# tlk00/BitMagic

Measured on AMD Instinct MI355X. Metric: Gbits/s + % HBM roofline, 256-way fused AND+COUNT on 1B-bit vectors, higher is better.
Workload: dtype u64; 1 GPU; aggregator pipeline combine_and_sub counts-only: 256-way AND+COUNT, 256 x 1000000000-bit vectors in total, data set A (common 10% OR noise 10%: no early exit); vectors=256, bits_per_vector=1000000000, density_q16=6554, blocks_per_vector=15259, blocks_per_rank=15259, hbm_resident_bytes=32279432448

## Files before the change

bitmagic_amd/_ffi.py:

```python
from __future__ import annotations

import ctypes as C
import os

_HERE = os.path.dirname(os.path.abspath(__file__))
LIB_PATH = os.environ.get("BMX_LIB") or os.path.join(_HERE, "lib", "libbmx.so")

OK, ERR_BADALLOC, ERR_BADARG, ERR_RANGE, ERR_DEVICE = 0, 1, 2, 3, 4
RC_BATCH_MAX = 8


class BmxError(RuntimeError):
    def __init__(self, status: int, msg: str, detail: str):
        super().__init__(f"{msg}" + (f" [{detail}]" if detail else ""))
        self.status = status


_lib = None


def lib() -> C.CDLL:
    global _lib
    if _lib is not None:
        return _lib
# ... 146 lines not shown
        "bmx_timer_stop_ms": (i32, [vp, P(C.c_float)]),
    }
    missing = []
    for name, (res, args) in sig.items():
        try:
            fn = getattr(L, name)
        except AttributeError:
            missing.append(name)
            continue
        fn.restype, fn.argtypes = res, args
    if missing:
        raise ImportError(f"libbmx.so does not export: {', '.join(missing)}")
    if hasattr(L, "bmx_diag_stream_read"):
        L.bmx_diag_stream_read.restype = i32
        L.bmx_diag_stream_read.argtypes = [vp, u64, i32, u32, i32, i32, P(C.c_float)]
    _lib = L
    return L


def exported_symbols():
    import re
    hdr = os.path.join(os.path.dirname(_HERE), "include", "bmx.h")
    txt = open(hdr).read()
    return sorted(set(re.findall(r"\b(bmx_[a-z0-9_]+)\s*\(", txt)))


def check(status: int) -> None:
    if status != OK:
        L = lib()
        raise BmxError(status, L.bmx_error_msg(status).decode(), L.bmx_last_error().decode())
# ... 1 lines not shown
```

bitmagic_amd/csrc/bmx.hip:

```cpp
#include "bmx_internal.h"
#ifdef BMX_DIAG
#include "bmx_diag.h"
#endif
#include "bmx_kernels2.h"
#include "bmx_kernels3.h"
#include "bmx_kernels4.h"
#include "bmx_kernels5.h"
#include "bmx_kernels6.h"
#include "bmx_kernels7.h"
#include "bmx_kernels8.h"
#include "bmx_kernels9.h"
#include "bmx_kernels10.h"
#include "bmx_kernels11.h"
#include "bmx_kernels12.h"
#include "bmx_kernels13.h"
#include "bmx_kernels14.h"
#include "bmx_kernels15.h"
#include "bmx_kernels16.h"
#include "bmx_kernels17.h"
#include "bmx_kernels18.h"

#include <algorithm>
#include <atomic>
#include <chrono>
// ... 734 lines not shown
#endif
#undef B2
    return nullptr;
}
static pipe_bits_fn pipe_bits_kernel(u32 rows, u32 unroll, bool nt, u32 wg)
{
    switch (rows) {
    case 8: return pipe_bits_rows<8>(unroll, nt, wg);
    case 4: return pipe_bits_rows<4>(unroll, nt, wg);
    case 2: return pipe_bits_rows<2>(unroll, nt, wg);
    case 1: return pipe_bits_rows<1>(unroll, nt, wg);
    default: return nullptr;
    }
}

static int ctx_set_tuning(bmx_ctx* ctx, const char* key, int value)
{
    ARGCHK(ctx && key);
    std::string k(key);
    if (k == "pipe_unroll") { ARGCHK(value == 0 || value == 1 || value == 2 || value == 4 || value == 8 || value == 16); ctx->pipe_unroll = value; }
    else if (k == "pipe_rows") { ARGCHK(value == 0 || value == 8 || value == 4 || value == 2 || value == 1); ctx->pipe_rows = value; }
    else if (k == "pipe_nt") ctx->pipe_nt = value != 0;
    else if (k == "pipe_lds") { ARGCHK(value >= 0 && value <= 160 * 1024); ctx->pipe_lds = value; }
    else if (k == "pipe_slots") { ARGCHK(value == 8 || value == 16); ctx->pipe_slots = value; }
    else if (k == "pipe_staged") { ARGCHK(value >= -1 && value <= 1); ctx->pipe_staged = value; }
    else if (k == "pipe_split") { ARGCHK(value >= -1 && value <= 1); ctx->pipe_split = value; }
    else if (k == "pipe_window") { ARGCHK(value >= -1); ctx->pipe_window = value; }
    else if (k == "or_tile") { ARGCHK(value >= 0 && value <= 3); ctx->or_tile = value; }
    else if (k == "or_rows") { ARGCHK(value >= -1 && value <= 1); ctx->or_rows = value; }
    else if (k == "or_depth") { ARGCHK(value == 4 || value == 8); ctx->or_depth = value; }
    else if (k == "direct_cols") { ARGCHK(value >= 0); ctx->direct_cols = value; }
    else if (k == "pair_stream") { ARGCHK(value == -1 || value == 0 || value == 2 || value == 4 || value == 8); ctx->pair_stream = value; }
    else if (k == "pair_wgs") { ARGCHK(value >= 1 && value <= 8); ctx->pair_wgs = value; }
    else if (k == "range_halves") { ARGCHK(value == 0 || value == 1); ctx->range_halves = value; }
    else if (k == "gap_count") { ARGCHK(value >= -1 && value <= 1); ctx->gap_count = value; }
    else if (k == "agg_shape") { ARGCHK(value == 0 || value == 1); ctx->agg_shape = value; }
    else if (k == "and_rows") { ARGCHK(value >= -1 && value <= 1); ctx->and_rows = value; }
    else if (k == "and_rows_wg") { ARGCHK(value == 128 || value == 256 || value == 512); ctx->and_rows_wg = value; }
    else if (k == "and_rows_depth") { ARGCHK(value == 2 || value == 3 || value == 4 || value == 8); ctx->and_rows_depth = value; }
    else if (k == "and_rows_nt") ctx->and_rows_nt = value != 0;
    else if (k == "and_rows_ipw") { ARGCHK(value >= 0 && value <= 64); ctx->and_rows_ipw = value; }
    else if (k == "ff_window") { ARGCHK(value >= -1); ctx->ff_window = value; }
// ... 151 lines not shown
    HIPCHK(hipMemsetAsync(ctx->d_done, 0, FOLD_DONE_WORDS * 4, ctx->stream));
    HIPCHK(hipMalloc((void**)&ctx->d_slots2, COUNT_SLOTS * COUNT_SLOT_STRIDE * sizeof(u64)));
    HIPCHK(hipMemsetAsync(ctx->d_slots2, 0, COUNT_SLOTS * COUNT_SLOT_STRIDE * sizeof(u64), ctx->stream));
    HIPCHK(hipMalloc((void**)&ctx->d_done2, FOLD_DONE_WORDS * 4));
    HIPCHK(hipMemsetAsync(ctx->d_done2, 0, FOLD_DONE_WORDS * 4, ctx->stream));
    HIPCHK(hipHostMalloc((void**)&ctx->h_pend, PEND_SLOTS * 8 * sizeof(u64)));
    HIPCHK(hipMalloc((void**)&ctx->d_cursor, 64));
    HIPCHK(hipMemsetAsync(ctx->d_cursor, 0, 64, ctx->stream));
    { int v = 0; if (hipDeviceGetAttribute(&v, hipDeviceAttributeMaxSharedMemoryPerBlock, device) == hipSuccess && v > 0) ctx->max_lds_bytes = (uint32_t)v; else (void)hipGetLastError(); }
    { size_t fr = 0, tot = 0; if (hipMemGetInfo(&fr, &tot) == hipSuccess && fr) ctx->pack_cap = (uint64_t)fr / 4; else (void)hipGetLastError(); }
    if (const char* e = getenv("BMX_DEBUG_REDZONE")) ctx->redzone = atoi(e) != 0;
    if (const char* e = getenv("BMX_PACK_MAX_MB")) { long long mb = atoll(e); if (mb >= 0) ctx->pack_cap = (uint64_t)mb << 20; }
    if (const char* e = getenv("BMX_POOL_MAX_MB")) { long long mb = atoll(e); if (mb >= 0) ctx->pool_cap = (uint64_t)mb << 20; }
    static const char* const env_keys[][2] = {
        {"BMX_PIPE_UNROLL", "pipe_unroll"}, {"BMX_PIPE_ROWS", "pipe_rows"}, {"BMX_PIPE_NT", "pipe_nt"},
        {"BMX_PIPE_WG", "pipe_wg"}, {"BMX_PIPE_WINDOW", "pipe_window"}, {"BMX_PIPE_SPLIT", "pipe_split"}, {"BMX_OR_TILE", "or_tile"}, {"BMX_OR_ROWS", "or_rows"}, {"BMX_OR_DEPTH", "or_depth"}, {"BMX_OR_WINDOW", "or_window"}, {"BMX_DIRECT_COLS", "direct_cols"}, {"BMX_FF_WINDOW", "ff_window"}, {"BMX_RC_BATCH", "rc_batch"}, {"BMX_GAP_COUNT", "gap_count"}, {"BMX_AND_ROWS", "and_rows"}, {"BMX_AGG_SHAPE", "agg_shape"}, {"BMX_AND_ROWS_WG", "and_rows_wg"}, {"BMX_AND_ROWS_DEPTH", "and_rows_depth"}, {"BMX_AND_ROWS_NT", "and_rows_nt"}, {"BMX_AND_ROWS_IPW", "and_rows_ipw"}, {"BMX_RANGE_HALVES", "range_halves"}, {"BMX_PAIR_STREAM", "pair_stream"}, {"BMX_PAIR_WGS", "pair_wgs"}, {"BMX_RS_LANES", "rs_lanes"}, {"BMX_RS_SELECT_TOP", "rs_select_top"}, {"BMX_RS_SELECT_SEL", "rs_select_sel"}, {"BMX_RS_LINES", "rs_lines"}, {"BMX_RS_SELECT_LINES", "rs_select_lines"}, {"BMX_RS_SDIR_SHIFT", "rs_sdir_shift"}, {"BMX_COLL_SHAPE", "coll_shape"}, {"BMX_COLL_WINDOW", "coll_window"}, {"BMX_COLL_SPLIT", "coll_split"}, {"BMX_COLL_BUILD", "coll_build"}, {"BMX_EQ_BIG", "eq_big"}, {"BMX_PAIR_LOOP", "pair_loop"}, {"BMX_PAIR_NT", "pair_nt"}, {"BMX_EQ_BIG_SHAPE", "eq_big_shape"}, {"BMX_OP2_WGS", "op2_wgs"}, {"BMX_OP2_LOOP", "op2_loop"}, {"BMX_OP2_NT", "op2_nt"}, {"BMX_GAP_PACK", "gap_pack"}, {"BMX_COLL_MEMBERS", "coll_members"}, {"BMX_XCD_SWIZZLE", "xcd_swizzle"}, {"BMX_RANKC_PATH", "rankc_path"}, {"BMX_HITS_TABLE_KB", "hits_table_kb"}};
    for (auto& kv : env_keys)
        if (const char* e = getenv(kv[0])) (void)ctx_set_tuning(ctx.get(), kv[1], atoi(e));
    g_last_error.clear();
    *out = ctx.release();
    return BMX_OK;
ABI_END }

int bmx_ctx_destroy(bmx_ctx* ctx) { ABI_TRY if (ctx) ctx_release(ctx); return BMX_OK; ABI_END }

int bmx_ctx_set_tuning(bmx_ctx* ctx, const char* key, int value) { ABI_TRY return ctx_set_tuning(ctx, key, value); ABI_END }

int bmx_probe_stream_rw(bmx_ctx* ctx, uint64_t bytes, int sets, int wgs_per_cu, int iters, float* ms_per_pass)
{ ABI_TRY
    ARGCHK(ctx && ms_per_pass && bytes >= 8192 && sets >= 1 && sets <= 8 && wgs_per_cu >= 1 && wgs_per_cu <= 8 && iters >= 1);
    int rc = set_dev(ctx); if (rc) return rc;
// ... 1226 lines not shown
        }
        return BMX_OK;
    }
    case CK_AND_ROWS:
        hipLaunchKernelGGL(and_rows_kernel<AR_COUNT>(ctx), dim3((u32)((pl.nitems + pl.ar_ipw - 1u) / pl.ar_ipw)), dim3(pl.ar_wg), pl.lds, ctx->stream,
                           (const u64*)p->d_dmat, row_off, and_n, sub_n, p->col_stride, ngroups, nb_from, (u32)pl.nitems, ctx->xcd_swz, (u64*)d_counts,
                           (uint4*)nullptr, (u64*)nullptr, (BlockStat*)nullptr, 0u, 0xFFFFFFFFu, and_rows_diag_bits(), pl.ar_ipw);
        break;
    case CK_GAPCOUNT:
        HIPCHK(hipFuncSetAttribute(reinterpret_cast<const void*>(k_pipe_counts_gapcount<false>), hipFuncAttributeMaxDynamicSharedMemorySize, (int)pl.lds));
        hipLaunchKernelGGL(HIP_KERNEL_NAME(k_pipe_counts_gapcount<false>), dim3((u32)pl.nitems), dim3(1024), pl.lds, ctx->stream,
                           p->d_dmat, row_off, and_n, sub_n, p->col_stride, ngroups, nb_from, (u32)pl.nitems, (u64*)d_counts,
                           (uint4*)nullptr, (u64*)nullptr, (BlockStat*)nullptr, 0u, 0xFFFFFFFFu);
        break;
    case CK_GENERAL: {
        auto fn = k_pipe_counts<1>;
        if (pl.unroll != 1) fn = pl.unroll == 2 ? k_pipe_counts<2> : k_pipe_counts<4>;
        for (u32 c0 = 0; c0 < pl.ncols; c0 += pl.win.per) {
            u32 nitems = std::min(pl.win.per, pl.ncols - c0) * ngroups;
            hipLaunchKernelGGL(fn, dim3((nitems + 3) / 4), dim3(256), pl.lds, ctx->stream,
                               p->d_dmat, row_off, and_n, sub_n, p->col_stride, ngroups, nb_from + c0, nitems, ctx->xcd_swz, (u64*)d_counts);
            KCHK();
        }
        return BMX_OK;
    }
    }
    KCHK();
    return BMX_OK;
}

extern "C" {

int bmx_pipeline_describe(bmx_ctx* ctx, bmx_pipeline* p, uint32_t nb_from, uint32_t nb_to, char* buf, size_t buf_len, uint32_t* n_launches)
{ ABI_TRY
    ARGCHK(ctx && p && p->ctx == ctx && buf && buf_len > 0);
    if (n_launches) *n_launches = 1;
    int rc = pipe_range(p, nb_from, nb_to); if (rc) return rc;
    bmx_coll *ca = nullptr, *cs = nullptr;
    if (!p->h_uids.empty() && ctx->gap_pack != 0 && p->cm_gen == ctx->coll_gen) (void)pipe_colls_valid(ctx, p, &ca, &cs);
    const CountsPlan pl = counts_plan(ctx, p, nb_from, nb_to, p->ngroups, coll_serve(p, ca));
    switch (pl.kernel) {
    case CK_COLL_APPLY: snprintf(buf, buf_len, "k_coll_apply<AND_COUNT,512> x 1 launch, %llu workgroups (packed collection of the operand set)", pl.nitems); break;
    case CK_COLL_MEMBERS: snprintf(buf, buf_len, "k_coll_members<AND_COUNT> x 1 launch, a wave per (column, group): %u x %u items (members of a packed collection)", pl.ncols, pl.ngroups); break;
    case CK_STAGED: snprintf(buf, buf_len, "k_pipe_counts_staged<%u> x 1 launch, %u workgroups", pl.slots, pl.ncols); break;
    case CK_SPLIT: snprintf(buf, buf_len, "k_pipe_split<2,%d> x 1 launch, %llu workgroups", SPLIT_WAVES, pl.nitems); break;
    case CK_AND_ROWS: snprintf(buf, buf_len, "k_agg_and_rows<COUNT,%u,%u> x 1 launch, %llu workgroups", pl.ar_wg, pl.ar_depth, pl.nitems); break;
// ... 2431 lines not shown
```

bitmagic_amd/csrc/bmx_device.h:

```cpp
#pragma once
#include <hip/hip_runtime.h>
#include <stdint.h>

typedef uint8_t  u8;
typedef uint16_t u16;
typedef uint32_t u32;
typedef uint64_t u64;

#define GMETA(e) ((u32)((e) >> 48) & 0x1FFFu)
#define GMETA_NONE 0xFFFFFFFFu
#define BMX_DESC_KIND(d) ((u32)((d) & 3ull))
#define BMX_DESC_PTR(d)  ((d) & ~3ull)

typedef u32 u32x4 __attribute__((ext_vector_type(4)));
typedef const __attribute__((address_space(1))) u32x4* gcptr4;
typedef __attribute__((address_space(1))) u32x4* gptr4;
typedef const __attribute__((address_space(1))) u16* gcptr16;

template <int ROWS> struct Part { u32x4 r[ROWS]; };
typedef Part<8> Blk;

__device__ __forceinline__ gcptr4 as_gc4(u64 addr) { return (gcptr4)(uintptr_t)addr; }
__device__ __forceinline__ gcptr4 as_gc4(const void* p) { return (gcptr4)(uintptr_t)p; }
__device__ __forceinline__ gptr4 as_g4(void* p) { return (gptr4)(uintptr_t)p; }
// ... 435 lines not shown
    const u32x4* l4 = reinterpret_cast<const u32x4*>(lds);
    u32 c = 0;
#pragma unroll
    for (int i = 0; i < 8; ++i) {
        u32x4 t = l4[i * 64 + lane];
        c += (u32)__popc(t.x) + (u32)__popc(t.y) + (u32)__popc(t.z) + (u32)__popc(t.w);
    }
    return uniform32(wave_sum(c));
}

#define SPARSE_CAP 1024u
#define SPARSE_NONE 0xFFFFFFFFu

struct GapStage { u32x4 d[3]; };

__device__ __forceinline__ void gap_stage_load(GapStage& s, gcptr16 g, u32 hdr, u32 lane)
{
    gcptr4 g4 = (gcptr4)(uintptr_t)g;
    u32 nch = ((hdr >> 3) + 8u) >> 3;
    const u32x4 z = {0u, 0u, 0u, 0u};
#pragma unroll
    for (int j = 0; j < 3; ++j) { u32 c = lane + 64u * (u32)j; s.d[j] = c < nch ? g4[c] : z; }
}
__device__ __forceinline__ void gap_stage_store(const GapStage& s, u32* lds, u32 hdr, u32 lane)
{
    u32x4* l4 = reinterpret_cast<u32x4*>(lds);
    u32 nch = ((hdr >> 3) + 8u) >> 3;
#pragma unroll
    for (int j = 0; j < 3; ++j) { u32 c = lane + 64u * (u32)j; if (c < nch) l4[c] = s.d[j]; }
}

template <int MODE, int NJ>
__device__ __forceinline__ u32 sparse_test(u32 (&cand)[16], const u16* G, u32 hdr)
{
    u32 len = hdr >> 3, sbit = hdr & 1u;
    u32 k[NJ];
#pragma unroll
    for (int j = 0; j < NJ; ++j) k[j] = 0u;
    for (u32 step = 1u << (31 - __builtin_clz(len)); step; step >>= 1) {
#pragma unroll
        for (int j = 0; j < NJ; ++j) {
            u32 t = k[j] + step; t = t < len ? t : len;
            u32 v = G[t];
            k[j] = v < cand[j] ? t : k[j];
        }
    }
#pragma unroll
    for (int j = 0; j < NJ; ++j) {
        u32 bitv = (sbit ^ k[j]) & 1u;
        bool keep = (MODE == GAP_AND) ? (bitv != 0u) : (bitv == 0u);
        if (!keep) cand[j] = SPARSE_NONE;
    }
    u32 alive = 0;
#pragma unroll
    for (int j = 0; j < NJ; ++j) alive += (u32)__popcll(__ballot(cand[j] != SPARSE_NONE));
    return alive;
}

template <int MODE>
__device__ __forceinline__ bool gap_apply_sparse(const u64* __restrict__ plist_back, u32 i0, u32 n, u32* lds, u32 lane)
{
    u16* list = reinterpret_cast<u16*>(lds + 640);
    u32 cand[16];
    u32 total, nj;
    {
        Blk b; blk_from_lds(b, lds, lane);
        __builtin_amdgcn_fence(__ATOMIC_ACQ_REL, "wavefront");
        __builtin_amdgcn_wave_barrier();
        u32 cnt = blk_lane_popcount(b);
        u32 incl = wave_scan_incl(cnt, lane);
        total = uniform32(__shfl(incl, 63, 64));
        u32 off = incl - cnt;
#pragma unroll
        for (int i = 0; i < 8; ++i) {
            u32 ws[4] = {b.r[i].x, b.r[i].y, b.r[i].z, b.r[i].w};
#pragma unroll
            for (int c = 0; c < 4; ++c) {
                u32 w = ws[c];
                u32 base = ((u32)i * 256u + lane * 4u + (u32)c) << 5;
                while (w) { u32 bit = (u32)__builtin_ctz(w); w &= w - 1u; list[off++] = (u16)(base + bit); }
            }
        }
        __builtin_amdgcn_fence(__ATOMIC_ACQ_REL, "wavefront");
        __builtin_amdgcn_wave_barrier();
        nj = (total + 63u) >> 6;
#pragma unroll
        for (int j = 0; j < 16; ++j) {
            u32 idx = (u32)j * 64u + lane;
            cand[j] = idx < total ? (u32)list[idx] : SPARSE_NONE;
        }
    }
    const u16* G = reinterpret_cast<const u16*>(lds);
    u32 i = i0;
    gcptr16 g0 = as_gc16(uniform64(*(plist_back - i)));
    u32 h0 = uniform32((u32)g0[0]);
    GapStage cur; gap_stage_load(cur, g0, h0, lane);
    gcptr16 g1 = as_gc16(uniform64(*(plist_back - (i + 1u < n ? i + 1u : n - 1u))));
    u32 h1v = (u32)g1[0];
    for (; i < n; ++i) {
        u32 h1 = uniform32(h1v);
        GapStage nxt; gap_stage_load(nxt, g1, h1, lane);
        u32 i2 = i + 2u < n ? i + 2u : n - 1u;
        gcptr16 g2 = as_gc16(uniform64(*(plist_back - i2)));
        u32 h2v = (u32)g2[0];
        gap_stage_store(cur, lds, h0, lane);
        __builtin_amdgcn_fence(__ATOMIC_ACQ_REL, "wavefront");
        __builtin_amdgcn_wave_barrier();
        u32 alive;
        if (nj <= 1u) alive = sparse_test<MODE, 1>(cand, G, h0);
        else if (nj <= 2u) alive = sparse_test<MODE, 2>(cand, G, h0);
        else if (nj <= 3u) alive = sparse_test<MODE, 3>(cand, G, h0);
        else if (nj <= 4u) alive = sparse_test<MODE, 4>(cand, G, h0);
        else if (nj <= 6u) alive = sparse_test<MODE, 6>(cand, G, h0);
        else if (nj <= 8u) alive = sparse_test<MODE, 8>(cand, G, h0);
        else if (nj <= 12u) alive = sparse_test<MODE, 12>(cand, G, h0);
        else alive = sparse_test<MODE, 16>(cand, G, h0);
        if (alive == 0u) return true;
        if (((alive + 63u) >> 6) < nj) {
            u32 mine = 0;
#pragma unroll
            for (int j = 0; j < 16; ++j) mine += cand[j] != SPARSE_NONE ? 1u : 0u;
            u32 off = wave_scan_incl(mine, lane) - mine;
#pragma unroll
            for (int j = 0; j < 16; ++j) if (cand[j] != SPARSE_NONE) list[off++] = (u16)cand[j];
            __builtin_amdgcn_fence(__ATOMIC_ACQ_REL, "wavefront");
            __builtin_amdgcn_wave_barrier();
            nj = (alive + 63u) >> 6;
#pragma unroll
            for (int j = 0; j < 16; ++j) {
                u32 idx = (u32)j * 64u + lane;
                cand[j] = idx < alive ? (u32)list[idx] : SPARSE_NONE;
            }
        }
        __builtin_amdgcn_fence(__ATOMIC_ACQ_REL, "wavefront");
        __builtin_amdgcn_wave_barrier();
        cur = nxt; g0 = g1; h0 = h1; g1 = g2; h1v = h2v;
    }
    {
        u32x4* l4 = reinterpret_cast<u32x4*>(lds);
        const u32x4 z = {0u, 0u, 0u, 0u};
#pragma unroll
        for (int r = 0; r < 8; ++r) l4[r * 64 + lane] = z;
        __builtin_amdgcn_fence(__ATOMIC_ACQ_REL, "wavefront");
        __builtin_amdgcn_wave_barrier();
#pragma unroll
        for (int j = 0; j < 16; ++j)
            if (cand[j] != SPARSE_NONE) atomicOr(&lds[cand[j] >> 5], 1u << (cand[j] & 31u));
        __builtin_amdgcn_fence(__ATOMIC_ACQ_REL, "wavefront");
        __builtin_amdgcn_wave_barrier();
    }
    return false;
}

template <int MODE>
__device__ __forceinline__ bool gap_apply_list(const u64* __restrict__ plist_back, u32 n, u32* lds, u32 lane)
{
    const bool CHECK = MODE != GAP_OR;
    u32 head = n >= 32u ? 8u : n;
    u32 i = 0;
    if constexpr (CHECK) {
        if (n >= 2u) {
            u32 pop = lds_blk_popcount(lds, lane);
            if (pop == 0u) return true;
            if (pop <= SPARSE_CAP) return gap_apply_sparse<MODE>(plist_back, 0u, n, lds, lane);
        }
    }
    for (; i < head; ++i) {
        gap_apply_lds_wave<MODE>(as_gc16(uniform64(*(plist_back - i))), lds, lane);
        if constexpr (CHECK) {
            __builtin_amdgcn_fence(__ATOMIC_ACQ_REL, "wavefront");
            __builtin_amdgcn_wave_barrier();
            u32 pop = lds_blk_popcount(lds, lane);
            if (pop == 0u) return true;
            if (pop <= SPARSE_CAP && i + 2u < n) return gap_apply_sparse<MODE>(plist_back, i + 1u, n, lds, lane);
        }
    }
    if (i < n) {
        u64 p = i + lane < n ? *(plist_back - (i + lane)) : 0ull;
        for (; i < n; i += 64u) {
            u64 pn = i + 64u + lane < n ? *(plist_back - (i + 64u + lane)) : 0ull;
            if (i + lane < n) gap_apply_lds_lane<MODE>(as_gc16(p), lds);
            p = pn;
            if constexpr (CHECK) {
                __builtin_amdgcn_fence(__ATOMIC_ACQ_REL, "wavefront");
                __builtin_amdgcn_wave_barrier();
                u32 pop = lds_blk_popcount(lds, lane);
                if (pop == 0u) return true;
                if (pop <= SPARSE_CAP && i + 64u + 2u <= n)
                    return gap_apply_sparse<MODE>(plist_back, i + 64u, n, lds, lane);
            }
        }
    }
    __builtin_amdgcn_fence(__ATOMIC_ACQ_REL, "wavefront");
    __builtin_amdgcn_wave_barrier();
    return false;
}

__device__ __forceinline__ u32 gap_lane_popcount(gcptr16 g, u32 lane, u32 meta = GMETA_NONE)
{
    u32 len, s;
    if (meta != GMETA_NONE) { len = meta >> 1; s = meta & 1u; }
    else { u32 hdr = g[0]; len = hdr >> 3; s = hdr & 1u; }
    u32 c = 0;
    for (u32 k = 1 + lane; k <= len; k += 64) {
// ... 75 lines not shown
```

bitmagic_amd/csrc/bmx_diag.h:

```cpp
#pragma once
#include "../../include/bmx.h"
#ifdef __cplusplus
extern "C" {
#endif
int bmx_diag_stream_read(bmx_ctx* ctx, uint64_t bytes, int nontemporal, uint32_t blocks_per_wave,
                         int pattern ,
                         int iters, float* ms_per_pass);
#ifdef __cplusplus
}
#endif
```

bitmagic_amd/csrc/bmx_internal.h:

```cpp
#pragma once
#include "../../include/bmx.h"
#include <hip/hip_runtime.h>
#include <stdint.h>

#include <map>
#include <memory>
#include <string>
#include <unordered_map>
#include <vector>

typedef uint8_t  u8;
typedef uint16_t u16;
typedef uint32_t u32;
typedef uint64_t u64;

int bmx_fail_hip(hipError_t e, const char* what, const char* file, int line);
void bmx_set_last_error(const char* msg);
#define HIPCHK(call) do { hipError_t e_ = (call); if (e_ != hipSuccess) return bmx_fail_hip(e_, #call, __FILE__, __LINE__); } while (0)
#define ARGCHK(cond) do { if (!(cond)) { bmx_set_last_error("bad argument: " #cond); return BMX_ERR_BADARG; } } while (0)
#define KCHK() HIPCHK(hipGetLastError())
#define PEND_SLOTS 1024
#include <new>
#include <stdexcept>
int bmx_abi_caught(int kind, const char* what);
// ... 24 lines not shown
    hipEvent_t ev_stage = nullptr;
    std::multimap<size_t, void*> pool_free;
    std::unordered_map<void*, size_t> pool_live;
    uint64_t pool_cached = 0, pool_cap = 16ull << 30;
    struct RzInfo { void* raw; size_t block; size_t bytes; int line; };
    bool redzone = false;
    std::unordered_map<void*, RzInfo> rz_live;
    uint64_t rz_hits = 0; std::string rz_report;
    long long fail_dmalloc_after = -1;
    bool fail_dmalloc_throws = false;
    int pipe_unroll = 0;
    int pipe_rows = 0;
    int pipe_nt = 1;
    int pipe_wg = 0;
    int pipe_window = 0;
    int pipe_staged = -1;
    int pipe_lds = 0;
    int pipe_slots = 16;
    int pipe_split = -1;
    int or_tile = 0;
    int direct_cols = 384;
    int pair_stream = -1;
    int pair_wgs = 1;
    int range_halves = 1;
    int gap_count = -1;
    int agg_shape = 0;
    int and_rows = -1;
    int and_rows_wg = 256;
    int and_rows_ipw = 0;
    int and_rows_nt = 0;
// ... 140 lines not shown
```

bitmagic_amd/csrc/bmx_kernels.h:

```cpp
#pragma once
#include "bmx_device.h"

#define DESC_MAKE(ptr, kind) ((u64)(uintptr_t)(ptr) | ((u64)(kind) << 62))
#define DESC_K(d) ((u32)((d) >> 62))
#define DESC_P(d) ((d) & 0x0000FFFFFFFFFFFFull)
#define DESC_MAKE_GAP(ptr, len, sbit) (DESC_MAKE(ptr, K_GAP) | ((u64)((((u32)(len)) << 1) | ((u32)(sbit) & 1u)) << 48))
enum { K_NULL = 0, K_FULL = 1, K_BIT = 2, K_GAP = 3 };

#define ROW_EMPTY 1ull
#define ROW_FULL  2ull
#define ROW_ONES  4ull

struct BlockStat { u32 pop; u32 runs; u32 first; u32 kind; };

__global__ __launch_bounds__(256)
void k_generate(u64 seed, u32 vec_id, int with_common, u32 d, u64 nbits, u64* __restrict__ out, u64 nwords64, u64 word0)
{
    u64 i = (u64)blockIdx.x * blockDim.x + threadIdx.x;
    u64 stride = (u64)gridDim.x * blockDim.x;
    for (; i < nwords64; i += stride) {
        u64 w = word0 + i;
        u64 v = gen_word64(seed, vec_id, w, d);
        if (with_common) v |= gen_word64(seed, 0xFFFFFFFFu, w, d);
        u64 bit0 = w * 64u;
// ... 344 lines not shown
    else if (!nbit && !ngap) { if (!sbit && !sgap) flags = ROW_FULL; else flags = ROW_ONES; }
    else if (!nbit) flags = ROW_ONES;
    if (lane == 0) {
        row[0] = (u64)nbit | ((u64)ngap << 16) | ((u64)sbit << 32) | ((u64)sgap << 48);
        row[1] = flags;
    }
}

__device__ __forceinline__ u32 xcd_remap(u32 b, u32 nwg)
{
    u32 q = nwg >> 3, rem = nwg & 7u;
    u32 x = b & 7u, i = b >> 3;
    return x * q + (x < rem ? x : rem) + i;
}

template <int U>
__global__ __launch_bounds__(256)
void k_pipe_counts(const u64* __restrict__ dmat, const u32* __restrict__ row_off,
                   const u32* __restrict__ and_n, const u32* __restrict__ sub_n, u32 col_stride,
                   u32 ngroups, u32 col_from, u32 nitems, int xcd_swz, u64* __restrict__ counts)
{
    extern __shared__ u32 lds_dyn[];
    u32 lane = lane_id(), wave = threadIdx.x >> 6;
    u32 bid = xcd_swz ? xcd_remap(blockIdx.x, gridDim.x) : blockIdx.x;
    u32 item = uniform32(bid * 4u + wave);
    if (item >= nitems) return;
    u32 c = item / ngroups, g = item - c * ngroups;
    const u64* row = dmat + (size_t)(col_from + c) * col_stride + row_off[g];
    u64 hdr = uniform64(row[0]), flags = uniform64(row[1]);
    if (flags & ROW_EMPTY) return;
    if (flags & ROW_FULL) { if (lane == 0) atomicAdd(reinterpret_cast<unsigned long long*>(&counts[g]), 65536ull); return; }
    u32 nba = (u32)(hdr & 0xFFFFu), nga = (u32)((hdr >> 16) & 0xFFFFu);
    u32 nbs = (u32)((hdr >> 32) & 0xFFFFu), ngs = (u32)(hdr >> 48);
    u32 na = uniform32(and_n[g]), ns = uniform32(sub_n[g]);
    const u64* pa = row + 2;
    const u64* ps = pa + na;
    u32* lds = lds_dyn + wave * 2048u;

    Blk acc;
    blk_fill(acc, ~0u);
    if (pipe_chain<U, true, 0>(acc, pa, nba, lane)) return;
    if (pipe_chain<U, true, 1>(acc, ps, nbs, lane)) return;
    if (nga | ngs) {
        blk_to_lds(acc, lds, lane);
        if (nga && gap_apply_list<GAP_AND>(pa + na - 1u, nga, lds, lane)) return;
        if (ngs && gap_apply_list<GAP_SUB>(ps + ns - 1u, ngs, lds, lane)) return;
        blk_from_lds(acc, lds, lane);
    }
    u32 cnt = wave_sum(blk_lane_popcount(acc));
    if (lane == 0 && cnt) atomicAdd(reinterpret_cast<unsigned long long*>(&counts[g]), (unsigned long long)cnt);
}

template <int U, bool NT, int WG = 256, int ROWS = 8>
__global__ __launch_bounds__(WG)
void k_pipe_counts_bits2(const u64* __restrict__ dmat, const u32* __restrict__ row_off,
                         const u32* __restrict__ and_n, u32 col_stride,
                         u32 ngroups, u32 col_from, u32 nitems, int xcd_swz, u64* __restrict__ counts)
{
    constexpr u32 PARTS = 8 / ROWS;
    u32 lane = lane_id(), wave = threadIdx.x >> 6, wpb = blockDim.x >> 6;
    u32 bid = xcd_swz ? xcd_remap(blockIdx.x, gridDim.x) : blockIdx.x;
    u32 item = uniform32(bid * wpb + wave);
    if (item >= nitems) return;
    u32 part = item % PARTS, cg = item / PARTS;
    u32 c = cg / ngroups, g = cg - c * ngroups;
    const u64* row = dmat + (size_t)(col_from + c) * col_stride + row_off[g];
// ... 96 lines not shown
```

bitmagic_amd/csrc/bmx_kernels2.h:

```cpp
#pragma once
#include "bmx_kernels.h"

enum { ST_OPT = 1, ST_FORCE_BIT = 2, ST_TEST_ZERO = 4, ST_TEST_ONE = 8, ST_FORCE_GAP = 16, ST_GAP_RESULT = 32 };

__device__ __forceinline__ void gap_emit_from_transitions(const Blk& t, u32 len, u32 first, u16* __restrict__ g, u32 lane, u16* __restrict__ stage)
{
    u32 idx_base = 1u;
#pragma unroll
    for (int i = 0; i < 8; ++i) {
        u32 c = __popc(t.r[i].x) + __popc(t.r[i].y) + __popc(t.r[i].z) + __popc(t.r[i].w);
        u32 incl = wave_scan_incl(c, lane);
        u32 idx = idx_base + incl - c;
        u32 wbase = (u32)i * 256u + lane * 4u;
        u32 tw[4] = {t.r[i].x, t.r[i].y, t.r[i].z, t.r[i].w};
#pragma unroll
        for (int j = 0; j < 4; ++j) {
            u32 m = tw[j];
            while (m) {
                u32 k = __builtin_ctz(m); m &= m - 1u;
                stage[idx++] = (u16)((wbase + j) * 32u + k - 1u);
            }
        }
        idx_base += __shfl(incl, 63, 64);
    }
// ... 907 lines not shown
    u32 c = col_from + blockIdx.x;
    if (tid < 8) cnt[tid] = 0u;
    if (MODE == DIRECT_FIND_FIRST) {
        if (tid == 0) cnt[5] = (((u64)c << 16) > __hip_atomic_load(best, __ATOMIC_RELAXED, __HIP_MEMORY_SCOPE_AGENT)) ? 1u : 0u;
        __syncthreads();
        if (cnt[5]) return;
    } else __syncthreads();
    for (u32 i = tid; i < n_and + n_sub; i += blockDim.x) {
        bool is_sub = i >= n_and;
        u32 nb = nblk[i];
        u64 d = c < nb ? descs[i][c] : 0ull;
        u32 k = DESC_K(d);
        if (MODE == DIRECT_OR) {
            if (k == K_FULL) cnt[4] = 1u;
            else if (k == K_BIT) { u32 p = atomicAdd(&cnt[0], 1u); bitA[p] = DESC_P(d); }
            else if (k == K_GAP) { u32 p = atomicAdd(&cnt[1], 1u); *(gapA - p) = DESC_P(d); }
        } else if (!is_sub) {
            if (k == K_NULL) cnt[4] = 1u;
            else if (k == K_BIT) { u32 p = atomicAdd(&cnt[0], 1u); bitA[p] = DESC_P(d); }
            else if (k == K_GAP) { u32 p = atomicAdd(&cnt[1], 1u); *(gapA - p) = DESC_P(d); }
        } else {
            if (k == K_FULL) cnt[4] = 1u;
            else if (k == K_BIT) { u32 p = atomicAdd(&cnt[2], 1u); bitS[p] = DESC_P(d); }
            else if (k == K_GAP) { u32 p = atomicAdd(&cnt[3], 1u); *(gapS - p) = DESC_P(d); }
        }
    }
    __syncthreads();
    const u32 nba = cnt[0], nga = cnt[1], nbs = cnt[2], ngs = cnt[3];
    const bool nothing = !(nba | nga | nbs | ngs);
    if (MODE == DIRECT_OR) {
        if (cnt[4]) { if (wave == 0) store_trivial(K_FULL, c, desc, st, lane); return; }
        if (nothing) { if (wave == 0) store_trivial(K_NULL, c, desc, st, lane); return; }
    } else {
        if (cnt[4]) { if (MODE == DIRECT_AND_SUB && wave == 0) store_trivial(K_NULL, c, desc, st, lane); return; }
        if (nothing) {
            if (MODE == DIRECT_AND_SUB) { if (wave == 0) store_trivial(K_FULL, c, desc, st, lane); }
            else if (tid == 0) atomicMin(reinterpret_cast<unsigned long long*>(best), ((unsigned long long)c << 16) + (has_mask ? mask_from : 0u));
            return;
        }
// ... 465 lines not shown
```

Baseline: 56300 Gbit/s.

## Deepen sparse GAP-list prefetch into a multi-stage ring with packed metadata

Reworks the sparse candidate-testing loop over GAP blocks so it prefetches entries with one wave-wide load and keeps a ring of D staged GAP blocks in flight, where the old loop looked only two blocks ahead. GAP list pointers now carry packed length/start-bit metadata taken from the descriptor, which removes a dependent header load before each block's staged copy. Out-of-range staging loads are clamped to the last chunk instead of being predicated. The aim is to hide the latency of dependent global loads in the sparse phase, at the cost of more registers for the ring. Also adds a tuning knob and a diagnostic phase-timing kernel.

```diff
diff --git a/bitmagic_amd/_ffi.py b/bitmagic_amd/_ffi.py
--- a/bitmagic_amd/_ffi.py
+++ b/bitmagic_amd/_ffi.py
@@ -184,6 +184,9 @@
     if hasattr(L, "bmx_diag_stream_read"):
         L.bmx_diag_stream_read.restype = i32
         L.bmx_diag_stream_read.argtypes = [vp, u64, i32, u32, i32, i32, P(C.c_float)]
+    if hasattr(L, "bmx_diag_pipe_phases"):
+        L.bmx_diag_pipe_phases.restype = i32
+        L.bmx_diag_pipe_phases.argtypes = [vp, vp, i32, vp, u64, P(u64), P(C.c_float)]
     _lib = L
     return L
 
diff --git a/bitmagic_amd/csrc/bmx.hip b/bitmagic_amd/csrc/bmx.hip
--- a/bitmagic_amd/csrc/bmx.hip
+++ b/bitmagic_amd/csrc/bmx.hip
@@ -772,6 +772,19 @@
     }
 }
 
+typedef void (*pipe_counts_fn)(const u64*, const u32*, const u32*, const u32*, u32, u32, u32, u32, int, u64*);
+template <int SD>
+static pipe_counts_fn pipe_counts_unroll(u32 unroll) { return unroll == 1 ? k_pipe_counts<1, SD> : unroll == 2 ? k_pipe_counts<2, SD> : k_pipe_counts<4, SD>; }
+static pipe_counts_fn pipe_counts_kernel(u32 unroll, int depth)
+{
+#ifdef BMX_TUNE
+    switch (depth) { case 1: return pipe_counts_unroll<1>(unroll); case 2: return pipe_counts_unroll<2>(unroll);
+                     case 4: return pipe_counts_unroll<4>(unroll); case 8: return pipe_counts_unroll<8>(unroll); default: break; }
+#endif
+    (void)depth;
+    return pipe_counts_unroll<BMX_SPARSE_DEPTH>(unroll);
+}
+
 static int ctx_set_tuning(bmx_ctx* ctx, const char* key, int value)
 {
     ARGCHK(ctx && key);
@@ -784,6 +797,14 @@
     else if (k == "pipe_staged") { ARGCHK(value >= -1 && value <= 1); ctx->pipe_staged = value; }
     else if (k == "pipe_split") { ARGCHK(value >= -1 && value <= 1); ctx->pipe_split = value; }
     else if (k == "pipe_window") { ARGCHK(value >= -1); ctx->pipe_window = value; }
+    else if (k == "sparse_depth") {
+#ifdef BMX_TUNE
+        ARGCHK(value == 0 || value == 1 || value == 2 || value == 4 || value == 8);
+#else
+        ARGCHK(value == 0 || value == BMX_SPARSE_DEPTH);
+#endif
+        ctx->sparse_depth = value;
+    }
     else if (k == "or_tile") { ARGCHK(value >= 0 && value <= 3); ctx->or_tile = value; }
     else if (k == "or_rows") { ARGCHK(value >= -1 && value <= 1); ctx->or_rows = value; }
     else if (k == "or_depth") { ARGCHK(value == 4 || value == 8); ctx->or_depth = value; }
@@ -965,7 +986,7 @@
     if (const char* e = getenv("BMX_POOL_MAX_MB")) { long long mb = atoll(e); if (mb >= 0) ctx->pool_cap = (uint64_t)mb << 20; }
     static const char* const env_keys[][2] = {
         {"BMX_PIPE_UNROLL", "pipe_unroll"}, {"BMX_PIPE_ROWS", "pipe_rows"}, {"BMX_PIPE_NT", "pipe_nt"},
-        {"BMX_PIPE_WG", "pipe_wg"}, {"BMX_PIPE_WINDOW", "pipe_window"}, {"BMX_PIPE_SPLIT", "pipe_split"}, {"BMX_OR_TILE", "or_tile"}, {"BMX_OR_ROWS", "or_rows"}, {"BMX_OR_DEPTH", "or_depth"}, {"BMX_OR_WINDOW", "or_window"}, {"BMX_DIRECT_COLS", "direct_cols"}, {"BMX_FF_WINDOW", "ff_window"}, {"BMX_RC_BATCH", "rc_batch"}, {"BMX_GAP_COUNT", "gap_count"}, {"BMX_AND_ROWS", "and_rows"}, {"BMX_AGG_SHAPE", "agg_shape"}, {"BMX_AND_ROWS_WG", "and_rows_wg"}, {"BMX_AND_ROWS_DEPTH", "and_rows_depth"}, {"BMX_AND_ROWS_NT", "and_rows_nt"}, {"BMX_AND_ROWS_IPW", "and_rows_ipw"}, {"BMX_RANGE_HALVES", "range_halves"}, {"BMX_PAIR_STREAM", "pair_stream"}, {"BMX_PAIR_WGS", "pair_wgs"}, {"BMX_RS_LANES", "rs_lanes"}, {"BMX_RS_SELECT_TOP", "rs_select_top"}, {"BMX_RS_SELECT_SEL", "rs_select_sel"}, {"BMX_RS_LINES", "rs_lines"}, {"BMX_RS_SELECT_LINES", "rs_select_lines"}, {"BMX_RS_SDIR_SHIFT", "rs_sdir_shift"}, {"BMX_COLL_SHAPE", "coll_shape"}, {"BMX_COLL_WINDOW", "coll_window"}, {"BMX_COLL_SPLIT", "coll_split"}, {"BMX_COLL_BUILD", "coll_build"}, {"BMX_EQ_BIG", "eq_big"}, {"BMX_PAIR_LOOP", "pair_loop"}, {"BMX_PAIR_NT", "pair_nt"}, {"BMX_EQ_BIG_SHAPE", "eq_big_shape"}, {"BMX_OP2_WGS", "op2_wgs"}, {"BMX_OP2_LOOP", "op2_loop"}, {"BMX_OP2_NT", "op2_nt"}, {"BMX_GAP_PACK", "gap_pack"}, {"BMX_COLL_MEMBERS", "coll_members"}, {"BMX_XCD_SWIZZLE", "xcd_swizzle"}, {"BMX_RANKC_PATH", "rankc_path"}, {"BMX_HITS_TABLE_KB", "hits_table_kb"}};
+        {"BMX_PIPE_WG", "pipe_wg"}, {"BMX_PIPE_WINDOW", "pipe_window"}, {"BMX_SPARSE_DEPTH", "sparse_depth"},{"BMX_PIPE_SPLIT", "pipe_split"}, {"BMX_OR_TILE", "or_tile"}, {"BMX_OR_ROWS", "or_rows"}, {"BMX_OR_DEPTH", "or_depth"}, {"BMX_OR_WINDOW", "or_window"}, {"BMX_DIRECT_COLS", "direct_cols"}, {"BMX_FF_WINDOW", "ff_window"}, {"BMX_RC_BATCH", "rc_batch"}, {"BMX_GAP_COUNT", "gap_count"}, {"BMX_AND_ROWS", "and_rows"}, {"BMX_AGG_SHAPE", "agg_shape"}, {"BMX_AND_ROWS_WG", "and_rows_wg"}, {"BMX_AND_ROWS_DEPTH", "and_rows_depth"}, {"BMX_AND_ROWS_NT", "and_rows_nt"}, {"BMX_AND_ROWS_IPW", "and_rows_ipw"}, {"BMX_RANGE_HALVES", "range_halves"}, {"BMX_PAIR_STREAM", "pair_stream"}, {"BMX_PAIR_WGS", "pair_wgs"}, {"BMX_RS_LANES", "rs_lanes"}, {"BMX_RS_SELECT_TOP", "rs_select_top"}, {"BMX_RS_SELECT_SEL", "rs_select_sel"}, {"BMX_RS_LINES", "rs_lines"}, {"BMX_RS_SELECT_LINES", "rs_select_lines"}, {"BMX_RS_SDIR_SHIFT", "rs_sdir_shift"}, {"BMX_COLL_SHAPE", "coll_shape"}, {"BMX_COLL_WINDOW", "coll_window"}, {"BMX_COLL_SPLIT", "coll_split"}, {"BMX_COLL_BUILD", "coll_build"}, {"BMX_EQ_BIG", "eq_big"}, {"BMX_PAIR_LOOP", "pair_loop"}, {"BMX_PAIR_NT", "pair_nt"}, {"BMX_EQ_BIG_SHAPE", "eq_big_shape"}, {"BMX_OP2_WGS", "op2_wgs"}, {"BMX_OP2_LOOP", "op2_loop"}, {"BMX_OP2_NT", "op2_nt"}, {"BMX_GAP_PACK", "gap_pack"}, {"BMX_COLL_MEMBERS", "coll_members"}, {"BMX_XCD_SWIZZLE", "xcd_swizzle"}, {"BMX_RANKC_PATH", "rankc_path"}, {"BMX_HITS_TABLE_KB", "hits_table_kb"}};
     for (auto& kv : env_keys)
         if (const char* e = getenv(kv[0])) (void)ctx_set_tuning(ctx.get(), kv[1], atoi(e));
     g_last_error.clear();
@@ -2222,8 +2243,7 @@
                            (uint4*)nullptr, (u64*)nullptr, (BlockStat*)nullptr, 0u, 0xFFFFFFFFu);
         break;
     case CK_GENERAL: {
-        auto fn = k_pipe_counts<1>;
-        if (pl.unroll != 1) fn = pl.unroll == 2 ? k_pipe_counts<2> : k_pipe_counts<4>;
+        const pipe_counts_fn fn = pipe_counts_kernel(pl.unroll, ctx->sparse_depth);
         for (u32 c0 = 0; c0 < pl.ncols; c0 += pl.win.per) {
             u32 nitems = std::min(pl.win.per, pl.ncols - c0) * ngroups;
             hipLaunchKernelGGL(fn, dim3((nitems + 3) / 4), dim3(256), pl.lds, ctx->stream,
@@ -2238,6 +2258,32 @@
 }
 
 extern "C" {
+
+#ifdef BMX_DIAG
+int bmx_diag_pipe_phases(bmx_ctx* ctx, bmx_pipeline* p, int depth, uint64_t* ticks, uint64_t n_items, uint64_t* count, float* ms)
+{ ABI_TRY
+    ARGCHK(ctx && p && p->ctx == ctx && ticks && count && ms && p->ngroups == 1 && n_items == p->ncols);
+    ARGCHK(depth == 1 || depth == 2 || depth == 4 || depth == 8);
+    int rc = set_dev(ctx); if (rc) return rc;
+    const u32 nitems = p->ncols;
+    DevBuf buf(ctx);
+    if ((rc = dmalloc(ctx, &buf.p, (size_t)nitems * 24))) return rc;
+    HIPCHK(hipMemsetAsync(buf.p, 0, (size_t)nitems * 24, ctx->stream));
+    HIPCHK(hipMemsetAsync(ctx->d_small, 0, 8, ctx->stream));
+    HIPCHK(hipEventRecord(ctx->ev0, ctx->stream));
+#define DIAG_PH(SD) hipLaunchKernelGGL(HIP_KERNEL_NAME(k_pipe_counts_diag<4, SD>), dim3((nitems + 3) / 4), dim3(256), 4 * 2048 * 4, ctx->stream, \
+        (const u64*)p->d_dmat, (const u32*)p->d_meta, (const u32*)p->d_meta + p->ngroups, (const u32*)p->d_meta + 2 * p->ngroups, p->col_stride, 1u, 0u, nitems, ctx->xcd_swz, (u64*)ctx->d_small, (u64*)buf.p)
+    switch (depth) { case 1: DIAG_PH(1); break; case 2: DIAG_PH(2); break; case 4: DIAG_PH(4); break; default: DIAG_PH(8); break; }
+#undef DIAG_PH
+    KCHK();
+    HIPCHK(hipEventRecord(ctx->ev1, ctx->stream));
+    HIPCHK(hipMemcpyAsync(ticks, buf.p, (size_t)nitems * 24, hipMemcpyDeviceToHost, ctx->stream));
+    HIPCHK(hipMemcpyAsync(count, ctx->d_small, 8, hipMemcpyDeviceToHost, ctx->stream));
+    HIPCHK(hipStreamSynchronize(ctx->stream));
+    HIPCHK(hipEventElapsedTime(ms, ctx->ev0, ctx->ev1));
+    return BMX_OK;
+ABI_END }
+#endif
 
 int bmx_pipeline_describe(bmx_ctx* ctx, bmx_pipeline* p, uint32_t nb_from, uint32_t nb_to, char* buf, size_t buf_len, uint32_t* n_launches)
 { ABI_TRY
diff --git a/bitmagic_amd/csrc/bmx_device.h b/bitmagic_amd/csrc/bmx_device.h
--- a/bitmagic_amd/csrc/bmx_device.h
+++ b/bitmagic_amd/csrc/bmx_device.h
@@ -473,26 +473,40 @@
 
 struct GapStage { u32x4 d[3]; };
 
-__device__ __forceinline__ void gap_stage_load(GapStage& s, gcptr16 g, u32 hdr, u32 lane)
+#ifndef BMX_SPARSE_DEPTH
+#define BMX_SPARSE_DEPTH 2
+#endif
+
+__device__ __forceinline__ void gap_stage_load(GapStage& s, gcptr16 g, u32 meta, u32 lane)
 {
     gcptr4 g4 = (gcptr4)(uintptr_t)g;
-    u32 nch = ((hdr >> 3) + 8u) >> 3;
-    const u32x4 z = {0u, 0u, 0u, 0u};
-#pragma unroll
-    for (int j = 0; j < 3; ++j) { u32 c = lane + 64u * (u32)j; s.d[j] = c < nch ? g4[c] : z; }
-}
-__device__ __forceinline__ void gap_stage_store(const GapStage& s, u32* lds, u32 hdr, u32 lane)
+    u32 nch = ((meta >> 1) + 8u) >> 3;
+#pragma unroll
+    for (int j = 0; j < 3; ++j) { u32 c = lane + 64u * (u32)j; s.d[j] = g4[c < nch ? c : nch - 1u]; }
+}
+template <int D>
+__device__ __forceinline__ u64 gap_entries_load(const u64* __restrict__ plist_back, u32 from, u32 last, u32 lane)
+{
+    u32 x = from + (lane < (u32)D ? lane : (u32)D - 1u);
+    return *(plist_back - (x < last ? x : last));
+}
+__device__ __forceinline__ u64 lane_entry(u64 v, int r)
+{
+    u32 lo = (u32)__builtin_amdgcn_readlane((int)(u32)v, r), hi = (u32)__builtin_amdgcn_readlane((int)(u32)(v >> 32), r);
+    return ((u64)hi << 32) | lo;
+}
+__device__ __forceinline__ void gap_stage_store(const GapStage& s, u32* lds, u32 meta, u32 lane)
 {
     u32x4* l4 = reinterpret_cast<u32x4*>(lds);
-    u32 nch = ((hdr >> 3) + 8u) >> 3;
+    u32 nch = ((meta >> 1) + 8u) >> 3;
 #pragma unroll
     for (int j = 0; j < 3; ++j) { u32 c = lane + 64u * (u32)j; if (c < nch) l4[c] = s.d[j]; }
 }
 
 template <int MODE, int NJ>
-__device__ __forceinline__ u32 sparse_test(u32 (&cand)[16], const u16* G, u32 hdr)
-{
-    u32 len = hdr >> 3, sbit = hdr & 1u;
+__device__ __forceinline__ u32 sparse_test(u32 (&cand)[16], const u16* G, u32 meta)
+{
+    u32 len = meta >> 1, sbit = meta & 1u;
     u32 k[NJ];
 #pragma unroll
     for (int j = 0; j < NJ; ++j) k[j] = 0u;
@@ -516,10 +530,29 @@
     return alive;
 }
 
-template <int MODE>
+__device__ __forceinline__ bool sparse_rebuild(const u32 (&cand)[16], u32* lds, u32 lane)
+{
+    u32x4* l4 = reinterpret_cast<u32x4*>(lds);
+    const u32x4 z = {0u, 0u, 0u, 0u};
+#pragma unroll
+    for (int r = 0; r < 8; ++r) l4[r * 64 + lane] = z;
+    __builtin_amdgcn_fence(__ATOMIC_ACQ_REL, "wavefront");
+    __builtin_amdgcn_wave_barrier();
+#pragma unroll
+    for (int j = 0; j < 16; ++j)
+        if (cand[j] != SPARSE_NONE) atomicOr(&lds[cand[j] >> 5], 1u << (cand[j] & 31u));
+    __builtin_amdgcn_fence(__ATOMIC_ACQ_REL, "wavefront");
+    __builtin_amdgcn_wave_barrier();
+    return false;
+}
+
+template <int MODE, int D>
 __device__ __forceinline__ bool gap_apply_sparse(const u64* __restrict__ plist_back, u32 i0, u32 n, u32* lds, u32 lane)
 {
     u16* list = reinterpret_cast<u16*>(lds + 640);
+    const u32 last = n - 1u;
+    const u64 e_first = gap_entries_load<D>(plist_back, i0, last, lane);
+    u64 e_next = gap_entries_load<D>(plist_back, i0 + (u32)D, last, lane);
     u32 cand[16];
     u32 total, nj;
     {
@@ -550,68 +583,65 @@
         }
     }
     const u16* G = reinterpret_cast<const u16*>(lds);
-    u32 i = i0;
-    gcptr16 g0 = as_gc16(uniform64(*(plist_back - i)));
-    u32 h0 = uniform32((u32)g0[0]);
-    GapStage cur; gap_stage_load(cur, g0, h0, lane);
-    gcptr16 g1 = as_gc16(uniform64(*(plist_back - (i + 1u < n ? i + 1u : n - 1u))));
-    u32 h1v = (u32)g1[0];
-    for (; i < n; ++i) {
-        u32 h1 = uniform32(h1v);
-        GapStage nxt; gap_stage_load(nxt, g1, h1, lane);
-        u32 i2 = i + 2u < n ? i + 2u : n - 1u;
-        gcptr16 g2 = as_gc16(uniform64(*(plist_back - i2)));
-        u32 h2v = (u32)g2[0];
-        gap_stage_store(cur, lds, h0, lane);
-        __builtin_amdgcn_fence(__ATOMIC_ACQ_REL, "wavefront");
-        __builtin_amdgcn_wave_barrier();
-        u32 alive;
-        if (nj <= 1u) alive = sparse_test<MODE, 1>(cand, G, h0);
-        else if (nj <= 2u) alive = sparse_test<MODE, 2>(cand, G, h0);
-        else if (nj <= 3u) alive = sparse_test<MODE, 3>(cand, G, h0);
-        else if (nj <= 4u) alive = sparse_test<MODE, 4>(cand, G, h0);
-        else if (nj <= 6u) alive = sparse_test<MODE, 6>(cand, G, h0);
-        else if (nj <= 8u) alive = sparse_test<MODE, 8>(cand, G, h0);
-        else if (nj <= 12u) alive = sparse_test<MODE, 12>(cand, G, h0);
-        else alive = sparse_test<MODE, 16>(cand, G, h0);
-        if (alive == 0u) return true;
-        if (((alive + 63u) >> 6) < nj) {
-            u32 mine = 0;
-#pragma unroll
-            for (int j = 0; j < 16; ++j) mine += cand[j] != SPARSE_NONE ? 1u : 0u;
-            u32 off = wave_scan_incl(mine, lane) - mine;
-#pragma unroll
-            for (int j = 0; j < 16; ++j) if (cand[j] != SPARSE_NONE) list[off++] = (u16)cand[j];
+    GapStage ring[D];
+    u32 rmeta[D];
+#pragma unroll
+    for (int r = 0; r < D; ++r) {
+        u64 e = lane_entry(e_first, r);
+        rmeta[r] = GMETA(e);
+        gap_stage_load(ring[r], as_gc16(e), rmeta[r], lane);
+        __builtin_amdgcn_sched_barrier(0);
+    }
+    for (u32 base = i0; base < n; base += (u32)D) {
+        const u64 e_cur = e_next;
+        e_next = gap_entries_load<D>(plist_back, base + 2u * (u32)D, last, lane);
+#pragma unroll
+        for (int r = 0; r < D; ++r) {
+            const u32 i = base + (u32)r;
+            if (i >= n) return sparse_rebuild(cand, lds, lane);
+            const u32 meta = rmeta[r];
+            gap_stage_store(ring[r], lds, meta, lane);
+            {
+                u64 e = lane_entry(e_cur, r);
+                rmeta[r] = GMETA(e);
+                gap_stage_load(ring[r], as_gc16(e), rmeta[r], lane);
+            }
             __builtin_amdgcn_fence(__ATOMIC_ACQ_REL, "wavefront");
             __builtin_amdgcn_wave_barrier();
-            nj = (alive + 63u) >> 6;
-#pragma unroll
-            for (int j = 0; j < 16; ++j) {
-                u32 idx = (u32)j * 64u + lane;
-                cand[j] = idx < alive ? (u32)list[idx] : SPARSE_NONE;
+            u32 alive;
+            if (nj <= 1u) alive = sparse_test<MODE, 1>(cand, G, meta);
+            else if (nj <= 2u) alive = sparse_test<MODE, 2>(cand, G, meta);
+            else if (nj <= 3u) alive = sparse_test<MODE, 3>(cand, G, meta);
+            else if (nj <= 4u) alive = sparse_test<MODE, 4>(cand, G, meta);
+            else if (nj <= 6u) alive = sparse_test<MODE, 6>(cand, G, meta);
+            else if (nj <= 8u) alive = sparse_test<MODE, 8>(cand, G, meta);
+            else if (nj <= 12u) alive = sparse_test<MODE, 12>(cand, G, meta);
+            else alive = sparse_test<MODE, 16>(cand, G, meta);
+            if (alive == 0u) return true;
+            if (((alive + 63u) >> 6) < nj) {
+                u32 mine = 0;
+#pragma unroll
+                for (int j = 0; j < 16; ++j) mine += cand[j] != SPARSE_NONE ? 1u : 0u;
+                u32 off = wave_scan_incl(mine, lane) - mine;
+#pragma unroll
+                for (int j = 0; j < 16; ++j) if (cand[j] != SPARSE_NONE) list[off++] = (u16)cand[j];
+                __builtin_amdgcn_fence(__ATOMIC_ACQ_REL, "wavefront");
+                __builtin_amdgcn_wave_barrier();
+                nj = (alive + 63u) >> 6;
+#pragma unroll
+                for (int j = 0; j < 16; ++j) {
+                    u32 idx = (u32)j * 64u + lane;
+                    cand[j] = idx < alive ? (u32)list[idx] : SPARSE_NONE;
+                }
             }
-        }
-        __builtin_amdgcn_fence(__ATOMIC_ACQ_REL, "wavefront");
-        __builtin_amdgcn_wave_barrier();
-        cur = nxt; g0 = g1; h0 = h1; g1 = g2; h1v = h2v;
-    }
-    {
-        u32x4* l4 = reinterpret_cast<u32x4*>(lds);
-        const u32x4 z = {0u, 0u, 0u, 0u};
-#pragma unroll
-        for (int r = 0; r < 8; ++r) l4[r * 64 + lane] = z;
-        __builtin_amdgcn_fence(__ATOMIC_ACQ_REL, "wavefront");
-        __builtin_amdgcn_wave_barrier();
-#pragma unroll
-        for (int j = 0; j < 16; ++j)
-            if (cand[j] != SPARSE_NONE) atomicOr(&lds[cand[j] >> 5], 1u << (cand[j] & 31u));
-        __builtin_amdgcn_fence(__ATOMIC_ACQ_REL, "wavefront");
-        __builtin_amdgcn_wave_barrier();
-    }
-    return false;
-}
-
-template <int MODE>
+            __builtin_amdgcn_fence(__ATOMIC_ACQ_REL, "wavefront");
+            __builtin_amdgcn_wave_barrier();
+        }
+    }
+    return sparse_rebuild(cand, lds, lane);
+}
+
+template <int MODE, int D = BMX_SPARSE_DEPTH>
 __device__ __forceinline__ bool gap_apply_list(const u64* __restrict__ plist_back, u32 n, u32* lds, u32 lane)
 {
     const bool CHECK = MODE != GAP_OR;
@@ -621,7 +651,7 @@
         if (n >= 2u) {
             u32 pop = lds_blk_popcount(lds, lane);
             if (pop == 0u) return true;
-            if (pop <= SPARSE_CAP) return gap_apply_sparse<MODE>(plist_back, 0u, n, lds, lane);
+            if (pop <= SPARSE_CAP) return gap_apply_sparse<MODE, D>(plist_back, 0u, n, lds, lane);
         }
     }
     for (; i < head; ++i) {
@@ -631,7 +661,7 @@
             __builtin_amdgcn_wave_barrier();
             u32 pop = lds_blk_popcount(lds, lane);
             if (pop == 0u) return true;
-            if (pop <= SPARSE_CAP && i + 2u < n) return gap_apply_sparse<MODE>(plist_back, i + 1u, n, lds, lane);
+            if (pop <= SPARSE_CAP && i + 2u < n) return gap_apply_sparse<MODE, D>(plist_back, i + 1u, n, lds, lane);
         }
     }
     if (i < n) {
@@ -646,7 +676,7 @@
                 u32 pop = lds_blk_popcount(lds, lane);
                 if (pop == 0u) return true;
                 if (pop <= SPARSE_CAP && i + 64u + 2u <= n)
-                    return gap_apply_sparse<MODE>(plist_back, i + 64u, n, lds, lane);
+                    return gap_apply_sparse<MODE, D>(plist_back, i + 64u, n, lds, lane);
             }
         }
     }
diff --git a/bitmagic_amd/csrc/bmx_diag.h b/bitmagic_amd/csrc/bmx_diag.h
--- a/bitmagic_amd/csrc/bmx_diag.h
+++ b/bitmagic_amd/csrc/bmx_diag.h
@@ -6,6 +6,8 @@
 int bmx_diag_stream_read(bmx_ctx* ctx, uint64_t bytes, int nontemporal, uint32_t blocks_per_wave,
                          int pattern ,
                          int iters, float* ms_per_pass);
+int bmx_diag_pipe_phases(bmx_ctx* ctx, bmx_pipeline* pipe, int depth , uint64_t* ticks, uint64_t n_items,
+                         uint64_t* count, float* ms);
 #ifdef __cplusplus
 }
 #endif
diff --git a/bitmagic_amd/csrc/bmx_internal.h b/bitmagic_amd/csrc/bmx_internal.h
--- a/bitmagic_amd/csrc/bmx_internal.h
+++ b/bitmagic_amd/csrc/bmx_internal.h
@@ -62,6 +62,7 @@
     int pipe_nt = 1;
     int pipe_wg = 0;
     int pipe_window = 0;
+    int sparse_depth = 0;
     int pipe_staged = -1;
     int pipe_lds = 0;
     int pipe_slots = 16;
diff --git a/bitmagic_amd/csrc/bmx_kernels.h b/bitmagic_amd/csrc/bmx_kernels.h
--- a/bitmagic_amd/csrc/bmx_kernels.h
+++ b/bitmagic_amd/csrc/bmx_kernels.h
@@ -382,17 +382,18 @@
     return x * q + (x < rem ? x : rem) + i;
 }
 
-template <int U>
-__global__ __launch_bounds__(256)
-void k_pipe_counts(const u64* __restrict__ dmat, const u32* __restrict__ row_off,
-                   const u32* __restrict__ and_n, const u32* __restrict__ sub_n, u32 col_stride,
-                   u32 ngroups, u32 col_from, u32 nitems, int xcd_swz, u64* __restrict__ counts)
+template <int U, int SD, bool DIAG>
+__device__ __forceinline__ void pipe_counts_item(const u64* __restrict__ dmat, const u32* __restrict__ row_off,
+                                                 const u32* __restrict__ and_n, const u32* __restrict__ sub_n, u32 col_stride,
+                                                 u32 ngroups, u32 col_from, u32 nitems, int xcd_swz, u64* __restrict__ counts,
+                                                 u64* __restrict__ diag)
 {
     extern __shared__ u32 lds_dyn[];
     u32 lane = lane_id(), wave = threadIdx.x >> 6;
     u32 bid = xcd_swz ? xcd_remap(blockIdx.x, gridDim.x) : blockIdx.x;
     u32 item = uniform32(bid * 4u + wave);
     if (item >= nitems) return;
+    if constexpr (DIAG) { if (lane == 0) diag[(size_t)item * 3u] = wall_clock64(); }
     u32 c = item / ngroups, g = item - c * ngroups;
     const u64* row = dmat + (size_t)(col_from + c) * col_stride + row_off[g];
     u64 hdr = uniform64(row[0]), flags = uniform64(row[1]);
@@ -409,15 +410,36 @@
     blk_fill(acc, ~0u);
     if (pipe_chain<U, true, 0>(acc, pa, nba, lane)) return;
     if (pipe_chain<U, true, 1>(acc, ps, nbs, lane)) return;
+    if constexpr (DIAG) { if (lane == 0) diag[(size_t)item * 3u + 1u] = wall_clock64(); }
     if (nga | ngs) {
         blk_to_lds(acc, lds, lane);
-        if (nga && gap_apply_list<GAP_AND>(pa + na - 1u, nga, lds, lane)) return;
-        if (ngs && gap_apply_list<GAP_SUB>(ps + ns - 1u, ngs, lds, lane)) return;
+        if (nga && gap_apply_list<GAP_AND, SD>(pa + na - 1u, nga, lds, lane)) { if constexpr (DIAG) { if (lane == 0) diag[(size_t)item * 3u + 2u] = wall_clock64(); } return; }
+        if (ngs && gap_apply_list<GAP_SUB, SD>(ps + ns - 1u, ngs, lds, lane)) { if constexpr (DIAG) { if (lane == 0) diag[(size_t)item * 3u + 2u] = wall_clock64(); } return; }
         blk_from_lds(acc, lds, lane);
     }
+    if constexpr (DIAG) { if (lane == 0) diag[(size_t)item * 3u + 2u] = wall_clock64(); }
     u32 cnt = wave_sum(blk_lane_popcount(acc));
     if (lane == 0 && cnt) atomicAdd(reinterpret_cast<unsigned long long*>(&counts[g]), (unsigned long long)cnt);
 }
+
+template <int U, int SD = BMX_SPARSE_DEPTH>
+__global__ __launch_bounds__(256)
+void k_pipe_counts(const u64* __restrict__ dmat, const u32* __restrict__ row_off,
+                   const u32* __restrict__ and_n, const u32* __restrict__ sub_n, u32 col_stride,
+                   u32 ngroups, u32 col_from, u32 nitems, int xcd_swz, u64* __restrict__ counts)
+{
+    pipe_counts_item<U, SD, false>(dmat, row_off, and_n, sub_n, col_stride, ngroups, col_from, nitems, xcd_swz, counts, nullptr);
+}
+#ifdef BMX_DIAG
+template <int U, int SD>
+__global__ __launch_bounds__(256)
+void k_pipe_counts_diag(const u64* __restrict__ dmat, const u32* __restrict__ row_off,
+                        const u32* __restrict__ and_n, const u32* __restrict__ sub_n, u32 col_stride,
+                        u32 ngroups, u32 col_from, u32 nitems, int xcd_swz, u64* __restrict__ counts, u64* __restrict__ diag)
+{
+    pipe_counts_item<U, SD, true>(dmat, row_off, and_n, sub_n, col_stride, ngroups, col_from, nitems, xcd_swz, counts, diag);
+}
+#endif
 
 template <int U, bool NT, int WG = 256, int ROWS = 8>
 __global__ __launch_bounds__(WG)
diff --git a/bitmagic_amd/csrc/bmx_kernels2.h b/bitmagic_amd/csrc/bmx_kernels2.h
--- a/bitmagic_amd/csrc/bmx_kernels2.h
+++ b/bitmagic_amd/csrc/bmx_kernels2.h
@@ -945,15 +945,15 @@
         if (MODE == DIRECT_OR) {
             if (k == K_FULL) cnt[4] = 1u;
             else if (k == K_BIT) { u32 p = atomicAdd(&cnt[0], 1u); bitA[p] = DESC_P(d); }
-            else if (k == K_GAP) { u32 p = atomicAdd(&cnt[1], 1u); *(gapA - p) = DESC_P(d); }
+            else if (k == K_GAP) { u32 p = atomicAdd(&cnt[1], 1u); *(gapA - p) = d & 0x3FFFFFFFFFFFFFFFull; }
         } else if (!is_sub) {
             if (k == K_NULL) cnt[4] = 1u;
             else if (k == K_BIT) { u32 p = atomicAdd(&cnt[0], 1u); bitA[p] = DESC_P(d); }
-            else if (k == K_GAP) { u32 p = atomicAdd(&cnt[1], 1u); *(gapA - p) = DESC_P(d); }
+            else if (k == K_GAP) { u32 p = atomicAdd(&cnt[1], 1u); *(gapA - p) = d & 0x3FFFFFFFFFFFFFFFull; }
         } else {
             if (k == K_FULL) cnt[4] = 1u;
             else if (k == K_BIT) { u32 p = atomicAdd(&cnt[2], 1u); bitS[p] = DESC_P(d); }
-            else if (k == K_GAP) { u32 p = atomicAdd(&cnt[3], 1u); *(gapS - p) = DESC_P(d); }
+            else if (k == K_GAP) { u32 p = atomicAdd(&cnt[3], 1u); *(gapS - p) = d & 0x3FFFFFFFFFFFFFFFull; }
         }
     }
     __syncthreads();
```

Result: no change. 56380 Gbit/s, median of 2 (+0.1%).
